# fixie-ai/ultravox

Hardware: NVIDIA H100
Metric: audio-sec/s prefill (Llama-3.1-8B, 30s clip) at 1/2/4/8 H100; TTFT p50 (higher is better)
Workload: dtype bf16

## Files before the change

### ultravox_b200/csrc/gemm_tc.cu

```cuda
#include <stdlib.h>

#include "uvx_common.cuh"
#include "tc_ptx.cuh"

namespace uvx {

struct GemmParams {
  int64_t a_rows, a_batch, K, N;
  void* C;
  int64_t c_row_stride, c_batch_rows, c_row_offset;
  const int32_t* c_row_map;
  const bf16* bias;
  const bf16* R;
  int64_t r_row_stride, r_batch_stride;
  float alpha;
  int act, out_f32;
  int m_tiles;
  int n_tiles, num_tiles;
  int splits, kb_per_split;
  float* ws_partial;
  const bf16* norm_w;
  bf16* norm_out;
  float norm_eps;
  int w_tiled;
  int w_perm;
  int swiglu;
  const float* rope_cos;
  const float* rope_sin;
  const int32_t* rope_pos;
  int64_t rope_rows_per_seq, rope_pos_offset;
  int rope_cols;
  int stages;
  int cm, cn;
};

static constexpr int kSmemTotal = 227 * 1024;
static constexpr int kMaxStages = 8;
static constexpr int kGemmThreads = 384;

template <int MT, int BN>
struct WgLayout {
  static constexpr int kABytes = MT * 128 * kBK * 2;
  static constexpr int kWBytes = BN * kBK * 2;
  static constexpr int kStageBytes = kABytes + kWBytes;
  static constexpr int kRingMax = kSmemTotal - 1024 - 256;
  static constexpr int kStages = kRingMax / kStageBytes > kMaxStages ? kMaxStages : kRingMax / kStageBytes;
  static constexpr int kAcc = BN / 2;
  static_assert(kStages >= 2, "ring too shallow");
  static_assert(MT * kAcc <= 128, "accumulators must fit the register file");
};

__device__ __forceinline__ int tile_col(int tc, int perm) {
  if (!perm) return tc;
  const int q = tc >> 5, j = tc & 31;
  return j < 16 ? 16 * q + j : 64 + 16 * q + (j - 16);
}

__device__ __forceinline__ int64_t out_row(const GemmParams& p, int b, int64_t m) {
  return p.c_row_map ? (int64_t)p.c_row_map[(int64_t)b * p.a_rows + m] : (int64_t)b * p.c_batch_rows + m + p.c_row_offset;
}

template <int BN, int I>
__device__ __forceinline__ void swiglu_row(const GemmParams& p, const float* a, int h, int cq, bf16* crow, int64_t n_out0) {
#pragma unroll
  for (int j = 0; j < BN / 8; ++j) {
    if ((8 * j) % (2 * I) >= I) continue;
    const int64_t f = n_out0 + (8 * j / (2 * I)) * I + (8 * j) % (2 * I) + cq;
    if (f >= p.N / 2) continue;
    constexpr int kUp = I / 8;
    float o[2];
#pragma unroll
    for (int e = 0; e < 2; ++e) {
      const float gate = __bfloat162float(__float2bfloat16_rn(a[4 * j + 2 * h + e] * p.alpha));
      const float up = __bfloat162float(__float2bfloat16_rn(a[4 * (j + kUp) + 2 * h + e] * p.alpha));
      o[e] = __bfloat162float(__float2bfloat16_rn(silu_fast(gate))) * up;
    }
    *reinterpret_cast<__nv_bfloat162*>(crow + f) = __floats2bfloat162_rn(o[0], o[1]);
  }
}

__device__ __forceinline__ void rope_store(const GemmParams& p, float x1a, float x1b, float x2a, float x2b, int64_t pos, int d, bf16* crow) {
  const float2 cs = *reinterpret_cast<const float2*>(p.rope_cos + pos * 64 + d);
  const float2 sn = *reinterpret_cast<const float2*>(p.rope_sin + pos * 64 + d);
  float o1a, o2a, o1b, o2b;
  rope_pair(__bfloat162float(__float2bfloat16_rn(x1a * p.alpha)), __bfloat162float(__float2bfloat16_rn(x2a * p.alpha)), cs.x, sn.x, o1a, o2a);
  rope_pair(__bfloat162float(__float2bfloat16_rn(x1b * p.alpha)), __bfloat162float(__float2bfloat16_rn(x2b * p.alpha)), cs.y, sn.y, o1b, o2b);
  *reinterpret_cast<__nv_bfloat162*>(crow + d) = __floats2bfloat162_rn(o1a, o1b);
  *reinterpret_cast<__nv_bfloat162*>(crow + d + 64) = __floats2bfloat162_rn(o2a, o2b);
}

template <int MT, int BN>
__global__ void __launch_bounds__(kGemmThreads, 1)
gemm_wg_kernel(const __grid_constant__ CUtensorMap tmA, const __grid_constant__ CUtensorMap tmW, const GemmParams p) {
  using L = WgLayout<MT, BN>;
  pdl_trigger();
  extern __shared__ uint8_t smem_raw[];
  uint8_t* smem = (uint8_t*)(((uintptr_t)smem_raw + 1023) & ~(uintptr_t)1023);
  uint64_t* full_bar = (uint64_t*)(smem + p.stages * L::kStageBytes);
  uint64_t* empty_bar = full_bar + kMaxStages;

  const int wg = threadIdx.x >> 7, tid = threadIdx.x & 127;
  const int tiles_m_total = p.m_tiles * (int)p.a_batch;
  const int num_kb = (int)((p.K + kBK - 1) / kBK);
  const int stages = p.stages;
  const int csize = p.cm * p.cn;
  const int rank = csize > 1 ? (int)cluster_ctarank() : 0;
  const int rm = rank / p.cn, rn = rank % p.cn;
  const int cluster_tiles_m = tiles_m_total / p.cm;
  const int num_units = p.num_tiles / csize * p.splits;
  const int first_unit = blockIdx.x / csize, unit_step = gridDim.x / csize;

  if (threadIdx.x == 0) {
    for (int s = 0; s < stages; ++s) {
      mbar_init(&full_bar[s], 1);
      mbar_init(&empty_bar[s], 8 * csize);
    }
    asm volatile("fence.mbarrier_init.release.cluster;" ::: "memory");
    asm volatile("fence.proxy.async.shared::cta;" ::: "memory");
  }
  if (csize > 1) cluster_sync();
  else __syncthreads();
  pdl_wait();

  if (wg == 0) {
    asm volatile("setmaxnreg.dec.sync.aligned.u32 40;");
    if (tid == 0) {
      asm volatile("prefetch.tensormap [%0];" ::"l"(&tmA) : "memory");
      asm volatile("prefetch.tensormap [%0];" ::"l"(&tmW) : "memory");
      const int a_slice = MT * 128 / p.cn, w_slice = BN / p.cm;
      const uint16_t row_mask = (uint16_t)(((1u << p.cn) - 1u) << (rm * p.cn));
      uint16_t col_mask = 0;
      for (int j = 0; j < p.cm; ++j) col_mask |= (uint16_t)(1u << (j * p.cn + rn));
      int s = 0;
      uint32_t ph = 0;
      for (int unit = first_unit; unit < num_units; unit += unit_step) {
        const int ctile = unit / p.splits, split = unit % p.splits;
        const int tm_idx = (ctile % cluster_tiles_m) * p.cm + rm;
        const int tn_idx = (ctile / cluster_tiles_m) * p.cn + rn;
        const int b = tm_idx / p.m_tiles;
        const int m0 = (tm_idx % p.m_tiles) * (MT * 128);
        const int kb_begin = split * p.kb_per_split;
        const int kb_end = min(num_kb, kb_begin + p.kb_per_split);
        const int wt_base = tn_idx * num_kb * BN;
        for (int kb = kb_begin; kb < kb_end; ++kb) {
          mbar_wait(&empty_bar[s], ph ^ 1u);
          uint8_t* sa = smem + s * L::kStageBytes;
          mbar_expect_tx(&full_bar[s], (uint32_t)L::kStageBytes);
          uint8_t* da = sa + rn * a_slice * (kBK * 2);
          if (p.cn > 1) tma_load_3d_mc(da, &tmA, kb * kBK, m0 + rn * a_slice, b, &full_bar[s], row_mask);
          else tma_load_3d(da, &tmA, kb * kBK, m0, b, &full_bar[s]);
          uint8_t* dw = sa + L::kABytes + rm * w_slice * (kBK * 2);
          const int w0 = p.w_tiled ? 0 : kb * kBK;
          const int w1 = (p.w_tiled ? wt_base + kb * BN : tn_idx * BN) + rm * w_slice;
          if (p.cm > 1) tma_load_2d_mc(dw, &tmW, w0, w1, &full_bar[s], col_mask);
          else tma_load_2d(dw, &tmW, w0, w1, &full_bar[s]);
          if (++s == stages) { s = 0; ph ^= 1u; }
        }
      }
    }
    if (csize > 1) cluster_sync();
    return;
  }

  asm volatile("setmaxnreg.inc.sync.aligned.u32 232;");
  const int c = wg - 1;
  const int warp = tid >> 5, lane = tid & 31;
  auto release = [&](int slot) {
    __syncwarp();
    if (csize == 1) {
      if (lane == 0) mbar_arrive(&empty_bar[slot]);
    } else if (lane < csize) {
// ... 25 lines not shown
#pragma unroll
        for (int k = 0; k < kBK / 16; ++k)
          Wgmma<BN>::mma(acc[mt], da + (uint64_t)(2 * k), dw + (uint64_t)(2 * k), (kb > kb_begin || k > 0) ? 1u : 0u);
      }
      wgmma_commit();
      wgmma_wait<1>();
      if (prev >= 0) release(prev);
      prev = s;
      if (++s == stages) { s = 0; ph ^= 1u; }
    }
    wgmma_wait<0>();
    release(prev);

    const int rq = warp * 16 + (lane >> 2);
    const int cq = 2 * (lane & 3);
    if (p.splits > 1) {
      float* part = p.ws_partial + (size_t)split * (size_t)(p.a_batch * p.a_rows) * (size_t)p.N;
#pragma unroll
      for (int mt = 0; mt < MT; ++mt) {
#pragma unroll
        for (int h = 0; h < 2; ++h) {
          const int64_t m = (int64_t)m0 + mt * 128 + c * 64 + rq + 8 * h;
          if (m >= p.a_rows) continue;
          float* dst = part + ((size_t)b * p.a_rows + m) * p.N;
#pragma unroll
          for (int j = 0; j < BN / 8; ++j) {
            const int64_t n = n0 + tile_col(8 * j + cq, p.w_perm);
            if (n < p.N) *reinterpret_cast<float2*>(dst + n) = make_float2(acc[mt][4 * j + 2 * h], acc[mt][4 * j + 2 * h + 1]);
          }
        }
      }
      continue;
    }
    if (p.swiglu) {
      const int64_t n_out0 = (int64_t)tn_idx * (BN / 2);
#pragma unroll
      for (int mt = 0; mt < MT; ++mt) {
#pragma unroll
        for (int h = 0; h < 2; ++h) {
          const int64_t m = (int64_t)m0 + mt * 128 + c * 64 + rq + 8 * h;
          if (m >= p.a_rows) continue;
          const int64_t orow = out_row(p, b, m);
          if (orow < 0) continue;
          bf16* crow = reinterpret_cast<bf16*>(p.C) + orow * p.c_row_stride;
          if (p.swiglu == 16) swiglu_row<BN, 16>(p, acc[mt], h, cq, crow, n_out0);
          else swiglu_row<BN, 8>(p, acc[mt], h, cq, crow, n_out0);
        }
      }
      continue;
    }
    if constexpr (BN == 128) {
      if (p.rope_cos != nullptr && n0 < p.rope_cols) {
#pragma unroll
        for (int mt = 0; mt < MT; ++mt) {
#pragma unroll
          for (int h = 0; h < 2; ++h) {
            const int64_t m = (int64_t)m0 + mt * 128 + c * 64 + rq + 8 * h;
            if (m >= p.a_rows) continue;
            const int64_t orow = out_row(p, b, m);
            if (orow < 0) continue;
            const int64_t pos = p.rope_pos ? (int64_t)p.rope_pos[m] : p.rope_pos_offset + (m % p.rope_rows_per_seq);
            bf16* crow = reinterpret_cast<bf16*>(p.C) + orow * p.c_row_stride + n0;
            const float* a = acc[mt];
            if (!p.w_perm) {
#pragma unroll
              for (int j = 0; j < 8; ++j)
                rope_store(p, a[4 * j + 2 * h], a[4 * j + 2 * h + 1], a[4 * (j + 8) + 2 * h], a[4 * (j + 8) + 2 * h + 1], pos, 8 * j + cq, crow);
            } else {
#pragma unroll
              for (int q = 0; q < 4; ++q)
#pragma unroll
                for (int jj = 0; jj < 2; ++jj) {
                  const int j = 4 * q + jj;
                  rope_store(p, a[4 * j + 2 * h], a[4 * j + 2 * h + 1], a[4 * (j + 2) + 2 * h], a[4 * (j + 2) + 2 * h + 1], pos,
                             16 * q + 8 * jj + cq, crow);
                }
            }
          }
        }
        continue;
      }
    }
#pragma unroll
    for (int mt = 0; mt < MT; ++mt) {
#pragma unroll
      for (int h = 0; h < 2; ++h) {
        const int64_t m = (int64_t)m0 + mt * 128 + c * 64 + rq + 8 * h;
        if (m >= p.a_rows) continue;
        const int64_t orow = out_row(p, b, m);
        if (orow < 0) continue;
        const bf16* rrow = p.R ? p.R + (int64_t)b * p.r_batch_stride + m * p.r_row_stride : nullptr;
#pragma unroll
        for (int j = 0; j < BN / 8; ++j) {
          const int64_t n = n0 + tile_col(8 * j + cq, p.w_perm);
          if (n >= p.N) continue;
          float v0 = acc[mt][4 * j + 2 * h] * p.alpha, v1 = acc[mt][4 * j + 2 * h + 1] * p.alpha;
          if (p.bias) {
            const float2 t = __bfloat1622float2(*reinterpret_cast<const __nv_bfloat162*>(p.bias + n));
            v0 += t.x;
            v1 += t.y;
          }
          if (p.act == UVX_ACT_GELU) {
            v0 = gelu_fast(v0);
            v1 = gelu_fast(v1);
          }
          if (rrow) {
            const float2 t = __bfloat1622float2(*reinterpret_cast<const __nv_bfloat162*>(rrow + n));
            v0 += t.x;
            v1 += t.y;
          }
          if (p.out_f32)
            *reinterpret_cast<float2*>(reinterpret_cast<float*>(p.C) + orow * p.c_row_stride + n) = make_float2(v0, v1);
          else
            *reinterpret_cast<__nv_bfloat162*>(reinterpret_cast<bf16*>(p.C) + orow * p.c_row_stride + n) = __floats2bfloat162_rn(v0, v1);
        }
      }
    }
  }
  if (csize > 1) cluster_sync();
}

__global__ void __launch_bounds__(256) splitk_reduce_kernel(const GemmParams p) {
  pdl_trigger();
  pdl_wait();
  const int64_t rows = p.a_batch * p.a_rows;
  const int64_t vec_per_row = p.N / 8;
  const int64_t total = rows * vec_per_row;
  const size_t split_stride = (size_t)rows * (size_t)p.N;
  for (int64_t idx = (int64_t)blockIdx.x * blockDim.x + threadIdx.x; idx < total; idx += (int64_t)gridDim.x * blockDim.x) {
    const int64_t r = idx / vec_per_row, n = (idx % vec_per_row) * 8;
    const int64_t b = r / p.a_rows, m = r % p.a_rows;
    const float* src = p.ws_partial + (size_t)r * p.N + n;
    float v[8] = {0.f, 0.f, 0.f, 0.f, 0.f, 0.f, 0.f, 0.f};
#pragma unroll 4
    for (int sidx = 0; sidx < p.splits; ++sidx) {
      const float4 t0 = __ldcg(reinterpret_cast<const float4*>(src + sidx * split_stride));
      const float4 t1 = __ldcg(reinterpret_cast<const float4*>(src + sidx * split_stride) + 1);
      v[0] += t0.x; v[1] += t0.y; v[2] += t0.z; v[3] += t0.w;
      v[4] += t1.x; v[5] += t1.y; v[6] += t1.z; v[7] += t1.w;
    }
    const int64_t orow = p.c_row_map ? (int64_t)p.c_row_map[r] : b * p.c_batch_rows + m + p.c_row_offset;
    if (orow < 0) continue;
#pragma unroll
    for (int i = 0; i < 8; ++i) v[i] *= p.alpha;
    if (p.bias) {
      float t[8];
      unpack8(*reinterpret_cast<const bf16x8*>(p.bias + n), t);
#pragma unroll
      for (int i = 0; i < 8; ++i) v[i] += t[i];
    }
    if (p.act == UVX_ACT_GELU) {
#pragma unroll
      for (int i = 0; i < 8; ++i) v[i] = gelu_erf(v[i]);
    }
    if (p.R) {
      float t[8];
      unpack8(*reinterpret_cast<const bf16x8*>(p.R + b * p.r_batch_stride + m * p.r_row_stride + n), t);
#pragma unroll
      for (int i = 0; i < 8; ++i) v[i] += t[i];
    }
    if (p.out_f32) {
      float4* dst = reinterpret_cast<float4*>(reinterpret_cast<float*>(p.C) + orow * p.c_row_stride + n);
      dst[0] = make_float4(v[0], v[1], v[2], v[3]);
      dst[1] = make_float4(v[4], v[5], v[6], v[7]);
    } else {
      *reinterpret_cast<bf16x8*>(reinterpret_cast<bf16*>(p.C) + orow * p.c_row_stride + n) = pack8(v);
    }
  }
}

__global__ void __launch_bounds__(256) splitk_reduce_rmsnorm_kernel(const GemmParams p) {
  pdl_trigger();
  pdl_wait();
  __shared__ float red[32];
  const int64_t r = blockIdx.x;
  const int64_t b = r / p.a_rows, m = r % p.a_rows;
  const int64_t rows = p.a_batch * p.a_rows;
  const size_t split_stride = (size_t)rows * (size_t)p.N;
  const int64_t orow = p.c_row_map ? (int64_t)p.c_row_map[r] : b * p.c_batch_rows + m + p.c_row_offset;
  constexpr int kMaxV = 4;
  float v[kMaxV][8];
  float sq = 0.f;
  const int nvec = (int)(p.N / 8);
#pragma unroll
  for (int i = 0; i < kMaxV; ++i) {
    const int j = threadIdx.x + i * 256;
    if (j < nvec) {
      const int64_t n = (int64_t)j * 8;
      const float* src = p.ws_partial + (size_t)r * p.N + n;
#pragma unroll
      for (int e = 0; e < 8; ++e) v[i][e] = 0.f;
      for (int s0 = 0; s0 < p.splits; s0 += 4) {
        float4 t0[4], t1[4];
#pragma unroll
        for (int u = 0; u < 4; ++u) {
          if (s0 + u < p.splits) {
            t0[u] = __ldcg(reinterpret_cast<const float4*>(src + (s0 + u) * split_stride));
            t1[u] = __ldcg(reinterpret_cast<const float4*>(src + (s0 + u) * split_stride) + 1);
          }
        }
#pragma unroll
        for (int u = 0; u < 4; ++u) {
// ... 179 lines not shown
}

typedef CUresult (*EncodeTiledFn)(CUtensorMap*, CUtensorMapDataType, cuuint32_t, void*, const cuuint64_t*,
                                  const cuuint64_t*, const cuuint32_t*, const cuuint32_t*, CUtensorMapInterleave,
                                  CUtensorMapSwizzle, CUtensorMapL2promotion, CUtensorMapFloatOOBfill);

static EncodeTiledFn get_encode() {
  static EncodeTiledFn fn = nullptr;
  if (!fn) {
    void* p = nullptr;
    cudaDriverEntryPointQueryResult q;
    if (cudaGetDriverEntryPoint("cuTensorMapEncodeTiled", &p, cudaEnableDefault, &q) == cudaSuccess &&
        q == cudaDriverEntryPointSuccess)
      fn = (EncodeTiledFn)p;
  }
  return fn;
}

static int encode_map(CUtensorMap* tm, const void* base, int rank, const uint64_t* dims, const uint64_t* strides_bytes,
                      const uint32_t* box, CUtensorMapL2promotion promo) {
  EncodeTiledFn enc = get_encode();
  if (!enc) {
    set_error("cuTensorMapEncodeTiled entry point not available");
    return UVX_ERR_CUDA;
  }
  cuuint64_t gd[3];
  cuuint64_t gs[2];
  cuuint32_t bx[3], es[3];
  for (int i = 0; i < rank; ++i) {
    gd[i] = dims[i];
    bx[i] = box[i];
    es[i] = 1;
  }
  for (int i = 0; i < rank - 1; ++i) gs[i] = strides_bytes[i];
  CUresult r = enc(tm, CU_TENSOR_MAP_DATA_TYPE_BFLOAT16, (cuuint32_t)rank, const_cast<void*>(base), gd, gs, bx, es,
                   CU_TENSOR_MAP_INTERLEAVE_NONE, CU_TENSOR_MAP_SWIZZLE_128B, promo, CU_TENSOR_MAP_FLOAT_OOB_FILL_NONE);
  if (r != CUDA_SUCCESS) {
    set_error("cuTensorMapEncodeTiled failed with CUresult %d (rank %d dims %llu %llu stride %llu)", (int)r, rank,
              (unsigned long long)dims[0], (unsigned long long)dims[1], (unsigned long long)strides_bytes[0]);
    return UVX_ERR_CUDA;
  }
  return UVX_OK;
}

static int num_sms() {
  static int n = 0;
  if (!n) {
    int dev = 0;
    cudaGetDevice(&dev);
    cudaDeviceGetAttribute(&n, cudaDevAttrMultiProcessorCount, dev);
    if (n <= 0) n = 132;
  }
  return n;
}

static int g_gemm_stage_cap = 0;
static int g_grid_cap = 0;

static int finish_gemm(const uvx_gemm_args* a, const GemmParams& p, cudaStream_t stream) {
  const bool want_norm = a->norm_w && a->norm_out;
  if (p.splits == 1) {
    if (!want_norm) return UVX_OK;
    return uvx_rmsnorm(a->C, a->norm_w, a->norm_out, a->a_batch * a->a_rows, a->N, a->c_row_stride, 0, 0, 0, a->norm_eps, stream);
  }
  if (want_norm && !p.out_f32 && a->N <= 8192 && !a->c_row_map && a->act == UVX_ACT_NONE) {
    launch_k(splitk_reduce_rmsnorm_kernel, dim3((unsigned)(a->a_batch * a->a_rows)), dim3(256), 0, stream, p);
    return check_launch("splitk_reduce_rmsnorm_kernel");
  }
  const int64_t total = a->a_batch * a->a_rows * (a->N / 8);
  int64_t blocks = (total + 255) / 256;
  if (blocks > (int64_t)num_sms() * 8) blocks = (int64_t)num_sms() * 8;
  launch_k(splitk_reduce_kernel, dim3((unsigned)blocks), dim3(256), 0, stream, p);
  int rc = check_launch("splitk_reduce_kernel");
  if (rc || !want_norm) return rc;
  return uvx_rmsnorm(a->C, a->norm_w, a->norm_out, a->a_batch * a->a_rows, a->N, a->c_row_stride, 0, 0, 0, a->norm_eps, stream);
}

static void legal_cluster(int mt, int bn, int tiles_m_total, int n_tiles, int* cm, int* cn) {
  if (*cm < 1 || *cm > 4 || tiles_m_total % *cm != 0 || bn % (8 * *cm) != 0) *cm = 1;
  if (*cn < 1 || *cn > 4 || n_tiles % *cn != 0 || (mt * 128) % (8 * *cn) != 0) *cn = 1;
  if (*cm * *cn > 8) *cm = *cn = 1;
}

template <int MT, int BN>
static int launch_gemm(const uvx_gemm_args* a, int splits, int cm, int cn, cudaStream_t stream) {
  using L = WgLayout<MT, BN>;
  const int m_tiles = (int)((a->a_rows + MT * 128 - 1) / (MT * 128));
  const int n_tiles = (int)((a->N + BN - 1) / BN);
  legal_cluster(MT, BN, m_tiles * (int)a->a_batch, n_tiles, &cm, &cn);
  CUtensorMap tmA, tmW;
  {
    uint64_t dims[3] = {(uint64_t)a->K, (uint64_t)a->a_rows, (uint64_t)a->a_batch};
    uint64_t st[2] = {(uint64_t)a->a_row_stride * 2, (uint64_t)(a->a_batch > 1 ? a->a_batch_stride : a->a_row_stride) * 2};
    uint32_t box[3] = {kBK, (uint32_t)(MT * 128 / cn), 1};
    int rc = encode_map(&tmA, a->A, 3, dims, st, box, CU_TENSOR_MAP_L2_PROMOTION_L2_128B);
    if (rc) return rc;
  }
  const bool tiled = a->w_tiled != 0;
  if (tiled) {
    UVX_REQUIRE(a->w_tiled == BN && a->K % kBK == 0, "uvx_gemm_bf16: tiled weights need BN == tile rows and K %% 64 == 0");
    const uint64_t n_tiles_w = (uint64_t)((a->N + BN - 1) / BN);
    uint64_t dims[2] = {(uint64_t)kBK, n_tiles_w * (uint64_t)(a->K / kBK) * (uint64_t)BN};
    uint64_t st[1] = {(uint64_t)kBK * 2};
    uint32_t box[2] = {kBK, (uint32_t)(BN / cm)};
    int rc = encode_map(&tmW, a->W, 2, dims, st, box, CU_TENSOR_MAP_L2_PROMOTION_L2_256B);
    if (rc) return rc;
  } else {
    uint64_t dims[2] = {(uint64_t)a->K, (uint64_t)a->N};
    uint64_t st[1] = {(uint64_t)a->w_row_stride * 2};
    uint32_t box[2] = {kBK, (uint32_t)(BN / cm)};
    int rc = encode_map(&tmW, a->W, 2, dims, st, box, CU_TENSOR_MAP_L2_PROMOTION_L2_256B);
    if (rc) return rc;
  }
  GemmParams p;
  memset(&p, 0, sizeof(p));
  p.w_tiled = tiled ? 1 : 0;
  p.w_perm = a->w_perm == 1 ? 1 : 0;
  p.swiglu = a->act == UVX_ACT_SWIGLU ? (a->w_tiled == 128 ? 16 : 8) : 0;
  p.rope_cos = a->rope_cos;
  p.rope_sin = a->rope_sin;
  p.rope_pos = a->rope_positions;
  p.rope_rows_per_seq = a->rope_rows_per_seq > 0 ? a->rope_rows_per_seq : 1;
  p.rope_pos_offset = a->rope_pos_offset;
  p.rope_cols = a->rope_cos ? (int)a->rope_cols : 0;
  if (p.swiglu || p.rope_cos || p.w_perm) splits = 1;
  p.a_rows = a->a_rows;
  p.a_batch = a->a_batch;
  p.K = a->K;
  p.N = a->N;
  p.C = a->C;
  p.c_row_stride = a->c_row_stride;
  p.c_batch_rows = a->c_batch_rows;
  p.c_row_offset = a->c_row_offset;
  p.c_row_map = a->c_row_map;
  p.bias = (const bf16*)a->bias;
  p.R = (const bf16*)a->R;
  p.r_row_stride = a->r_row_stride;
  p.r_batch_stride = a->r_batch_stride;
  p.alpha = a->alpha;
  p.act = a->act;
  p.out_f32 = a->out_dtype == UVX_DT_F32;
  p.norm_w = (const bf16*)a->norm_w;
  p.norm_out = (bf16*)a->norm_out;
  p.norm_eps = a->norm_eps;
  p.m_tiles = m_tiles;
  p.n_tiles = n_tiles;
  p.num_tiles = p.m_tiles * (int)a->a_batch * p.n_tiles;
  p.cm = cm;
  p.cn = cn;
  const int num_kb = (int)((a->K + kBK - 1) / kBK);
  if (a->N % BN != 0) splits = 1;
  const size_t per_split = (size_t)a->a_batch * (size_t)a->a_rows * (size_t)a->N * 4;
  while (splits > 1 && (!a->workspace || per_split * (size_t)splits > (size_t)a->workspace_bytes)) --splits;
  if (splits > num_kb) splits = num_kb;
  if (splits < 1) splits = 1;
  p.kb_per_split = (num_kb + splits - 1) / splits;
  p.splits = (num_kb + p.kb_per_split - 1) / p.kb_per_split;
  p.ws_partial = (float*)a->workspace;
  p.stages = L::kStages;
  if (g_gemm_stage_cap >= 2 && p.stages > g_gemm_stage_cap) p.stages = g_gemm_stage_cap;
  const int smem = p.stages * L::kStageBytes + 1024 + 2 * kMaxStages * 8;
  static bool attr_set = false;
  if (!attr_set) {
    cudaError_t e = cudaFuncSetAttribute(gemm_wg_kernel<MT, BN>, cudaFuncAttributeMaxDynamicSharedMemorySize, kSmemTotal);
    if (e != cudaSuccess) {
      set_error("cudaFuncSetAttribute(gemm_wg_kernel<%d,%d>, smem %d): %s", MT, BN, kSmemTotal, cudaGetErrorString(e));
      return UVX_ERR_CUDA;
    }
    attr_set = true;
  }
  const int csize = cm * cn;
  const int units = p.num_tiles / csize * p.splits;
  int max_units = num_sms();
  if (csize > 1) {
    static int max_clusters[9] = {0};
    if (!max_clusters[csize]) {
      cudaLaunchConfig_t cfg = {};
      cfg.gridDim = dim3((unsigned)csize);
      cfg.blockDim = dim3(kGemmThreads);
      cfg.dynamicSmemBytes = (size_t)smem;
      cudaLaunchAttribute attr;
      attr.id = cudaLaunchAttributeClusterDimension;
      attr.val.clusterDim.x = (unsigned)csize;
      attr.val.clusterDim.y = 1;
      attr.val.clusterDim.z = 1;
      cfg.attrs = &attr;
      cfg.numAttrs = 1;
      cudaError_t e = cudaOccupancyMaxActiveClusters(&max_clusters[csize], gemm_wg_kernel<MT, BN>, &cfg);
      if (e != cudaSuccess || max_clusters[csize] < 1) {
        set_error("cudaOccupancyMaxActiveClusters(gemm_wg_kernel<%d,%d>, %d CTAs): %s", MT, BN, csize,
                  e != cudaSuccess ? cudaGetErrorString(e) : "no cluster fits");
        max_clusters[csize] = 0;
        return UVX_ERR_CUDA;
      }
    }
    max_units = max_clusters[csize];
  }
  int clusters = units < max_units ? units : max_units;
  if (g_grid_cap > 0 && clusters * csize > g_grid_cap) clusters = g_grid_cap / csize > 1 ? g_grid_cap / csize : 1;
  const dim3 grid((unsigned)(clusters * csize));
  if (csize > 1)
    launch_k_cluster(gemm_wg_kernel<MT, BN>, grid, dim3(kGemmThreads), (size_t)smem, stream, (unsigned)csize, tmA, tmW, p);
  else
    launch_k(gemm_wg_kernel<MT, BN>, grid, dim3(kGemmThreads), (size_t)smem, stream, tmA, tmW, p);
  int rc = check_launch("gemm_wg_kernel");
  if (rc) return rc;
  return finish_gemm(a, p, stream);
}

static int g_ws_enable = -1;

static int gemm_ws_enabled() {
  if (g_ws_enable < 0) {
    const char* e = getenv("UVX_GEMM_WS");
    g_ws_enable = e ? atoi(e) : 2;
  }
  return g_ws_enable;
}

static bool gemm_ws_common(const uvx_gemm_args* a) {
  if (!gemm_ws_enabled() || (a->flags & 2)) return false;
  if (a->a_batch != 1 || a->out_dtype != UVX_DT_BF16 || a->c_row_map || a->c_row_offset != 0) return false;
  return a->w_tiled == 0 || a->w_tiled == 128;
}

static bool gemm_swap_eligible(const uvx_gemm_args* a) {
  if (!gemm_ws_common(a) || a->a_rows > 32 || a->act == UVX_ACT_SWIGLU) return false;
  return a->workspace && (size_t)a->workspace_bytes >= (size_t)a->a_rows * (size_t)a->N * 4;
}

static bool gemm_ws_eligible(const uvx_gemm_args* a) {
  return gemm_ws_common(a) && gemm_ws_enabled() == 1 && a->a_rows <= 256 && a->N % 128 == 0;
}

template <int BT>
static int launch_gemm_swap(const uvx_gemm_args* a, cudaStream_t stream) {
  constexpr int kStage = 128 * kBK * 2 + BT * kBK * 2;
  CUtensorMap tmX, tmW;
  {
    uint64_t dims[2] = {(uint64_t)a->K, (uint64_t)a->a_rows};
    uint64_t st[1] = {(uint64_t)a->a_row_stride * 2};
    uint32_t box[2] = {kBK, (uint32_t)BT};
    int rc = encode_map(&tmX, a->A, 2, dims, st, box, CU_TENSOR_MAP_L2_PROMOTION_L2_128B);
    if (rc) return rc;
  }
  const int num_kb = (int)((a->K + kBK - 1) / kBK);
  const int n_tiles = (int)((a->N + 127) / 128);
  if (a->w_tiled) {
    UVX_REQUIRE(a->K % kBK == 0, "uvx_gemm_bf16: tiled weights need K %% 64 == 0");
    uint64_t dims[2] = {(uint64_t)kBK, (uint64_t)n_tiles * (uint64_t)num_kb * 128};
    uint64_t st[1] = {(uint64_t)kBK * 2};
    uint32_t box[2] = {kBK, 128};
    int rc = encode_map(&tmW, a->W, 2, dims, st, box, CU_TENSOR_MAP_L2_PROMOTION_L2_256B);
    if (rc) return rc;
  } else {
    uint64_t dims[2] = {(uint64_t)a->K, (uint64_t)a->N};
    uint64_t st[1] = {(uint64_t)a->w_row_stride * 2};
    uint32_t box[2] = {kBK, 128};
    int rc = encode_map(&tmW, a->W, 2, dims, st, box, CU_TENSOR_MAP_L2_PROMOTION_L2_256B);
    if (rc) return rc;
  }
  GemmParams p;
  memset(&p, 0, sizeof(p));
  p.a_rows = a->a_rows;
  p.a_batch = 1;
  p.K = a->K;
  p.N = a->N;
  p.C = a->C;
  p.c_row_stride = a->c_row_stride;
  p.c_batch_rows = a->a_rows;
  p.bias = (const bf16*)a->bias;
  p.R = (const bf16*)a->R;
  p.r_row_stride = a->r_row_stride;
  p.r_batch_stride = a->r_batch_stride;
  p.alpha = a->alpha;
  p.act = a->act;
  p.norm_w = (const bf16*)a->norm_w;
  p.norm_out = (bf16*)a->norm_out;
  p.norm_eps = a->norm_eps;
  p.w_tiled = a->w_tiled ? 1 : 0;
  p.w_perm = a->w_perm == 1 ? 1 : 0;
  p.rope_cos = a->rope_cos;
  p.rope_sin = a->rope_sin;
  p.rope_pos = a->rope_positions;
  p.rope_rows_per_seq = a->rope_rows_per_seq > 0 ? a->rope_rows_per_seq : 1;
  p.rope_pos_offset = a->rope_pos_offset;
  p.rope_cols = a->rope_cos ? (int)a->rope_cols : 0;
  p.n_tiles = n_tiles;
  p.num_tiles = n_tiles;
  const int sms = num_sms();
  int splits = 1;
  if (n_tiles * 2 <= sms && num_kb >= 16) {
    splits = sms / n_tiles;
    if (splits > num_kb / 8) splits = num_kb / 8;
    if (splits > 16) splits = 16;
    if (splits < 1) splits = 1;
  }
  if (a->N % 8 != 0) splits = 1;
  const size_t per_split = (size_t)a->a_rows * (size_t)a->N * 4;
  while (splits > 1 && per_split * (size_t)splits > (size_t)a->workspace_bytes) --splits;
  p.kb_per_split = (num_kb + splits - 1) / splits;
  p.splits = (num_kb + p.kb_per_split - 1) / p.kb_per_split;
  p.ws_partial = (float*)a->workspace;
  p.stages = (kSmemTotal - 1024 - 256) / kStage;
  if (p.stages > kMaxStages) p.stages = kMaxStages;
  if (g_gemm_stage_cap >= 2 && p.stages > g_gemm_stage_cap) p.stages = g_gemm_stage_cap;
  const int smem = p.stages * kStage + 1024 + 2 * kMaxStages * 8;
  static bool attr_set = false;
  if (!attr_set) {
    cudaError_t e = cudaFuncSetAttribute(gemm_swap_kernel<BT>, cudaFuncAttributeMaxDynamicSharedMemorySize, kSmemTotal);
    if (e != cudaSuccess) {
      set_error("cudaFuncSetAttribute(gemm_swap_kernel<%d>): %s", BT, cudaGetErrorString(e));
      return UVX_ERR_CUDA;
    }
    attr_set = true;
  }
  const int units = n_tiles * p.splits;
  int grid = units < sms ? units : sms;
  if (g_grid_cap > 0 && grid > g_grid_cap) grid = g_grid_cap;
  launch_k(gemm_swap_kernel<BT>, dim3((unsigned)grid), dim3(kGemmThreads), (size_t)smem, stream, tmX, tmW, p);
  int rc = check_launch("gemm_swap_kernel");
  if (rc) return rc;
  if (p.rope_cos) {
    const int64_t total = a->a_rows * (a->N / 128) * 8;
    const int64_t blocks = (total + 255) / 256;
    launch_k(splitk_reduce_rope_kernel, dim3((unsigned)blocks), dim3(256), 0, stream, p);
    return check_launch("splitk_reduce_rope_kernel");
  }
  return finish_gemm(a, p, stream);
}

}

static int forced = -1, forced_splits = -1;

extern "C" int uvx_debug_gemm_override(int cfg, int splits) {
  forced = cfg;
  forced_splits = splits;
  return UVX_OK;
}

extern "C" int uvx_debug_gemm_stages(int n) {
  uvx::g_gemm_stage_cap = n;
  return UVX_OK;
}

extern "C" int uvx_debug_gemm_ws(int enable, int mode, int grid) {
  (void)mode;
  uvx::g_ws_enable = enable;
  uvx::g_grid_cap = grid > 0 ? grid : 0;
  return UVX_OK;
}

static int forced_cm = 0, forced_cn = 0;
static int g_cluster_enable = -1;

extern "C" int uvx_debug_gemm_cluster(int cm, int cn) {
  forced_cm = cm;
  forced_cn = cn;
  return UVX_OK;
}

extern "C" int uvx_debug_gemm_mode(int mode) { (void)mode; return UVX_OK; }
extern "C" int uvx_debug_gemm_tma_store(int on) { (void)on; return UVX_OK; }
extern "C" int uvx_debug_gemm_times(void* dev_buf) { (void)dev_buf; return UVX_OK; }
extern "C" int uvx_debug_gemm_pf(int pf) { (void)pf; return UVX_OK; }
extern "C" int uvx_debug_gemm_ws_times(void* dev_buf) { (void)dev_buf; return UVX_OK; }

static void read_forced() {
  if (forced < 0) {
    const char* e = getenv("UVX_GEMM_CFG");
    forced = e ? atoi(e) : 0;
    const char* s = getenv("UVX_GEMM_SPLITS");
    forced_splits = s ? atoi(s) : 0;
  }
}

static void pick_cfg(int64_t rows, int64_t batch, int64_t N, int64_t K, int sms, int* mt_out, int* bn_out, int* splits) {
  const int num_kb = (int)((K + 63) / 64);
  int mt, bn;
  if (rows <= 256 && batch == 1) {
    mt = rows > 128 ? 2 : 1;
    bn = N % 128 == 0 ? 128 : 64;
    if (bn == 128 && 2 * (N / 128) >= (sms * 3) / 5 && N / 128 < sms && num_kb <= 80) mt = 1;
  } else {
    mt = 1;
    const int64_t m_tiles = (rows + 127) / 128 * batch;
    if (N % 256 == 0 && m_tiles * (N / 256) >= sms && num_kb >= 32) bn = 256;
    else bn = (N % 128 == 0 && m_tiles * (N / 128) >= sms / 2) ? 128 : 64;
  }
  const int64_t tiles = ((rows + mt * 128 - 1) / (mt * 128)) * batch * ((N + bn - 1) / bn);
  int sp = 1;
  if (tiles * 2 <= sms && num_kb >= 16) {
    sp = (int)(sms / tiles);
    if (sp > num_kb / 8) sp = num_kb / 8;
    if (sp > 16) sp = 16;
    if (sp < 1) sp = 1;
  }
  *mt_out = mt;
  *bn_out = bn;
  *splits = sp;
}

static void pick_cluster(int64_t rows, int64_t batch, int mt, int* cm, int* cn) {
  *cm = *cn = 1;
  if (g_cluster_enable < 0) {
    const char* e = getenv("UVX_GEMM_CLUSTER");
    g_cluster_enable = e ? atoi(e) : 1;
  }
  if (forced_cm > 0 || forced_cn > 0) {
    *cm = forced_cm > 0 ? forced_cm : 1;
    *cn = forced_cn > 0 ? forced_cn : 1;
    return;
  }
  if (!g_cluster_enable || rows > 256 || batch != 1) return;
  if (mt == 1 && rows > 128) {
    *cm = 2;
    *cn = 2;
  }
}

extern "C" int uvx_gemm_bf16(const uvx_gemm_args* a, uvx_stream_t stream_) {
  using namespace uvx;
  cudaStream_t stream = (cudaStream_t)stream_;
  UVX_REQUIRE(a && a->A && a->W && a->C, "uvx_gemm_bf16: null pointer");
  UVX_REQUIRE(a->a_batch >= 1 && a->a_rows >= 1 && a->K >= 8 && a->N >= 64, "uvx_gemm_bf16: empty problem");
  UVX_REQUIRE(a->K % 8 == 0 && a->N % 64 == 0, "uvx_gemm_bf16: K %% 8 and N %% 64 required (K=%lld N=%lld)",
              (long long)a->K, (long long)a->N);
  UVX_REQUIRE(a->a_row_stride % 8 == 0 && a->w_row_stride % 8 == 0 && (a->a_batch == 1 || a->a_batch_stride % 8 == 0),
              "uvx_gemm_bf16: strides must be multiples of 8 elements");
  UVX_REQUIRE(((uintptr_t)a->A % 16 == 0) && ((uintptr_t)a->W % 16 == 0) && ((uintptr_t)a->C % 16 == 0),
              "uvx_gemm_bf16: 16-byte aligned bases required");
  UVX_REQUIRE(a->c_row_stride % 8 == 0 && (!a->R || (a->r_row_stride % 8 == 0 && a->r_batch_stride % 8 == 0)),
              "uvx_gemm_bf16: output / residual strides must be multiples of 8");
  UVX_REQUIRE(a->a_rows < (1ll << 31) && a->K < (1ll << 31) && a->N < (1ll << 31), "uvx_gemm_bf16: dimension too large");
  UVX_REQUIRE(!a->workspace || (uintptr_t)a->workspace % 256 == 0, "uvx_gemm_bf16: workspace must be 256-byte aligned");
  UVX_REQUIRE(!(a->norm_w && a->norm_out) || (a->out_dtype == UVX_DT_BF16 && !a->c_row_map && a->c_row_offset == 0 &&
                                              (a->a_batch == 1 || a->c_batch_rows == a->a_rows)),
              "uvx_gemm_bf16: fused RMSNorm needs a plain bf16 output");
  UVX_REQUIRE(a->w_tiled == 0 || a->w_tiled == 64 || a->w_tiled == 128 || a->w_tiled == 208 || a->w_tiled == 256,
              "uvx_gemm_bf16: w_tiled must be 64 / 128 / 208 / 256");
  UVX_REQUIRE(a->w_perm == 0 || (a->w_perm == 1 && a->w_tiled == 128 && a->N % 128 == 0 && a->act != UVX_ACT_SWIGLU),
              "uvx_gemm_bf16: the pair-permuted image (w_perm = 1) is a 128-row image of whole heads");
  UVX_REQUIRE(a->act != UVX_ACT_SWIGLU || (a->w_tiled != 0 && !a->bias && !a->R && !a->norm_w && a->out_dtype == UVX_DT_BF16 &&
                                           a->N % (a->w_tiled == 128 ? 32 : 16) == 0),
              "uvx_gemm_bf16: UVX_ACT_SWIGLU needs the interleaved gate|up image, bf16 output, no bias / residual / norm");
  UVX_REQUIRE(!a->rope_cos || (a->rope_sin && a->a_batch == 1 && a->alpha == 1.0f && !a->bias && !a->R && a->act == UVX_ACT_NONE &&
                               a->rope_cols % 128 == 0 && (a->w_tiled == 0 || a->w_tiled == 128) && a->N % 128 == 0),
              "uvx_gemm_bf16: fused RoPE needs head_dim 128 tiles, a_batch 1, no bias / residual / activation");
  read_forced();
  const int sms = num_sms();
  int mt, bn, splits;
  pick_cfg(a->a_rows, a->a_batch, a->N, a->K, sms, &mt, &bn, &splits);
  if (forced <= 0 && forced_splits <= 0 && gemm_swap_eligible(a)) {
    if (a->a_rows <= 8) return launch_gemm_swap<8>(a, stream);
    if (a->a_rows <= 16) return launch_gemm_swap<16>(a, stream);
    return launch_gemm_swap<32>(a, stream);
  }
  const bool ws = forced <= 0 && forced_splits <= 0 && gemm_ws_eligible(a);
  if (ws) {
    mt = 1;
    bn = 128;
    splits = 1;
  } else if (forced > 0) {
    const int fb = forced % 1000, fm = forced / 1000;
    if (fb == 64 || fb == 128 || fb == 208 || fb == 256) {
      if (a->N % fb == 0 || fb == 208) bn = fb;
      mt = fm == 2 ? 2 : 1;
    }
  }
  if (forced_splits > 0 && !ws) splits = forced_splits;
  if (a->w_tiled) bn = (int)a->w_tiled;
  if (a->rope_cos) {
    mt = 1;
    bn = 128;
  }
  if (bn > 128) mt = 1;
  int cm, cn;
  pick_cluster(a->a_rows, a->a_batch, mt, &cm, &cn);
  switch (mt * 1000 + bn) {
    case 1064: return launch_gemm<1, 64>(a, splits, cm, cn, stream);
    case 1128: return launch_gemm<1, 128>(a, splits, cm, cn, stream);
    case 1208: return launch_gemm<1, 208>(a, splits, cm, cn, stream);
    case 1256: return launch_gemm<1, 256>(a, splits, cm, cn, stream);
    case 2064: return launch_gemm<2, 64>(a, splits, cm, cn, stream);
    case 2128: return launch_gemm<2, 128>(a, splits, cm, cn, stream);
    default: return launch_gemm<1, 64>(a, splits, cm, cn, stream);
  }
}
```

Before: 1411.

## Add ping-pong warp-specialized GEMM kernel with heuristic tile selection

Adds a persistent GEMM kernel in which two consumer warpgroups alternate between output tiles, ordered by named barriers, so one warpgroup's epilogue overlaps the other's MMA main loop. A single TMA producer warpgroup feeds a shared smem ring. A heuristic picks 64x256 or 128x128 tiles when the per-SM wave work is lower than the cooperative kernel's, and only for plain GEMMs (no SwiGLU, RoPE, tiled weights or split-K). The plain epilogue is factored into a shared helper. Risks include extra register pressure from per-warpgroup accumulators and wrong pipeline phase tracking if the tile interleaving assumptions break.

```diff
diff --git a/ultravox_b200/csrc/gemm_tc.cu b/ultravox_b200/csrc/gemm_tc.cu
--- a/ultravox_b200/csrc/gemm_tc.cu
+++ b/ultravox_b200/csrc/gemm_tc.cu
@@ -87,6 +87,42 @@
   rope_pair(__bfloat162float(__float2bfloat16_rn(x1b * p.alpha)), __bfloat162float(__float2bfloat16_rn(x2b * p.alpha)), cs.y, sn.y, o1b, o2b);
   *reinterpret_cast<__nv_bfloat162*>(crow + d) = __floats2bfloat162_rn(o1a, o1b);
   *reinterpret_cast<__nv_bfloat162*>(crow + d + 64) = __floats2bfloat162_rn(o2a, o2b);
+}
+
+template <int BN>
+__device__ __forceinline__ void plain_epilogue(const GemmParams& p, const float* acc, int b, int64_t m_sub0, int n0, int rq, int cq) {
+#pragma unroll
+  for (int h = 0; h < 2; ++h) {
+    const int64_t m = m_sub0 + rq + 8 * h;
+    if (m >= p.a_rows) continue;
+    const int64_t orow = out_row(p, b, m);
+    if (orow < 0) continue;
+    const bf16* rrow = p.R ? p.R + (int64_t)b * p.r_batch_stride + m * p.r_row_stride : nullptr;
+#pragma unroll
+    for (int j = 0; j < BN / 8; ++j) {
+      const int64_t n = n0 + tile_col(8 * j + cq, p.w_perm);
+      if (n >= p.N) continue;
+      float v0 = acc[4 * j + 2 * h] * p.alpha, v1 = acc[4 * j + 2 * h + 1] * p.alpha;
+      if (p.bias) {
+        const float2 t = __bfloat1622float2(*reinterpret_cast<const __nv_bfloat162*>(p.bias + n));
+        v0 += t.x;
+        v1 += t.y;
+      }
+      if (p.act == UVX_ACT_GELU) {
+        v0 = gelu_fast(v0);
+        v1 = gelu_fast(v1);
+      }
+      if (rrow) {
+        const float2 t = __bfloat1622float2(*reinterpret_cast<const __nv_bfloat162*>(rrow + n));
+        v0 += t.x;
+        v1 += t.y;
+      }
+      if (p.out_f32)
+        *reinterpret_cast<float2*>(reinterpret_cast<float*>(p.C) + orow * p.c_row_stride + n) = make_float2(v0, v1);
+      else
+        *reinterpret_cast<__nv_bfloat162*>(reinterpret_cast<bf16*>(p.C) + orow * p.c_row_stride + n) = __floats2bfloat162_rn(v0, v1);
+    }
+  }
 }
 
 template <int MT, int BN>
@@ -278,42 +314,127 @@
       }
     }
 #pragma unroll
-    for (int mt = 0; mt < MT; ++mt) {
-#pragma unroll
-      for (int h = 0; h < 2; ++h) {
-        const int64_t m = (int64_t)m0 + mt * 128 + c * 64 + rq + 8 * h;
-        if (m >= p.a_rows) continue;
-        const int64_t orow = out_row(p, b, m);
-        if (orow < 0) continue;
-        const bf16* rrow = p.R ? p.R + (int64_t)b * p.r_batch_stride + m * p.r_row_stride : nullptr;
-#pragma unroll
-        for (int j = 0; j < BN / 8; ++j) {
-          const int64_t n = n0 + tile_col(8 * j + cq, p.w_perm);
-          if (n >= p.N) continue;
-          float v0 = acc[mt][4 * j + 2 * h] * p.alpha, v1 = acc[mt][4 * j + 2 * h + 1] * p.alpha;
-          if (p.bias) {
-            const float2 t = __bfloat1622float2(*reinterpret_cast<const __nv_bfloat162*>(p.bias + n));
-            v0 += t.x;
-            v1 += t.y;
-          }
-          if (p.act == UVX_ACT_GELU) {
-            v0 = gelu_fast(v0);
-            v1 = gelu_fast(v1);
-          }
-          if (rrow) {
-            const float2 t = __bfloat1622float2(*reinterpret_cast<const __nv_bfloat162*>(rrow + n));
-            v0 += t.x;
-            v1 += t.y;
-          }
-          if (p.out_f32)
-            *reinterpret_cast<float2*>(reinterpret_cast<float*>(p.C) + orow * p.c_row_stride + n) = make_float2(v0, v1);
-          else
-            *reinterpret_cast<__nv_bfloat162*>(reinterpret_cast<bf16*>(p.C) + orow * p.c_row_stride + n) = __floats2bfloat162_rn(v0, v1);
+    for (int mt = 0; mt < MT; ++mt) plain_epilogue<BN>(p, acc[mt], b, (int64_t)m0 + mt * 128 + c * 64, n0, rq, cq);
+  }
+  if (csize > 1) cluster_sync();
+}
+
+template <int TM, int TN>
+struct PpLayout {
+  static constexpr int kABytes = TM * kBK * 2;
+  static constexpr int kWBytes = TN * kBK * 2;
+  static constexpr int kStageBytes = kABytes + kWBytes;
+  static constexpr int kRingMax = kSmemTotal - 1024 - 256;
+  static constexpr int kStages = kRingMax / kStageBytes > kMaxStages ? kMaxStages : kRingMax / kStageBytes;
+  static constexpr int kSub = TM / 64;
+  static constexpr int kAcc = TN / 2;
+  static_assert(kStages >= 2, "ring too shallow");
+  static_assert(kSub * kAcc <= 128, "accumulators must fit the register file");
+};
+
+__device__ __forceinline__ void named_bar_sync(int id, int threads) {
+  asm volatile("bar.sync %0, %1;" ::"r"(id), "r"(threads) : "memory");
+}
+__device__ __forceinline__ void named_bar_arrive(int id, int threads) {
+  asm volatile("bar.arrive %0, %1;" ::"r"(id), "r"(threads) : "memory");
+}
+
+template <int TM, int TN>
+__global__ void __launch_bounds__(kGemmThreads, 1)
+gemm_pp_kernel(const __grid_constant__ CUtensorMap tmA, const __grid_constant__ CUtensorMap tmW, const GemmParams p) {
+  using L = PpLayout<TM, TN>;
+  pdl_trigger();
+  extern __shared__ uint8_t smem_raw[];
+  uint8_t* smem = (uint8_t*)(((uintptr_t)smem_raw + 1023) & ~(uintptr_t)1023);
+  uint64_t* full_bar = (uint64_t*)(smem + p.stages * L::kStageBytes);
+  uint64_t* empty_bar = full_bar + kMaxStages;
+
+  const int wg = threadIdx.x >> 7, tid = threadIdx.x & 127;
+  const int tiles_m_total = p.m_tiles * (int)p.a_batch;
+  const int num_kb = (int)((p.K + kBK - 1) / kBK);
+  const int stages = p.stages;
+  const int n_local = (p.num_tiles - (int)blockIdx.x + (int)gridDim.x - 1) / (int)gridDim.x;
+
+  if (threadIdx.x == 0) {
+    for (int s = 0; s < stages; ++s) {
+      mbar_init(&full_bar[s], 1);
+      mbar_init(&empty_bar[s], 4);
+    }
+    asm volatile("fence.mbarrier_init.release.cluster;" ::: "memory");
+    asm volatile("fence.proxy.async.shared::cta;" ::: "memory");
+  }
+  __syncthreads();
+  pdl_wait();
+
+  if (wg == 0) {
+    asm volatile("setmaxnreg.dec.sync.aligned.u32 40;");
+    if (tid == 0) {
+      asm volatile("prefetch.tensormap [%0];" ::"l"(&tmA) : "memory");
+      asm volatile("prefetch.tensormap [%0];" ::"l"(&tmW) : "memory");
+      int s = 0;
+      uint32_t ph = 0;
+      for (int i = 0; i < n_local; ++i) {
+        const int t = (int)blockIdx.x + i * (int)gridDim.x;
+        const int tm_idx = t % tiles_m_total, tn_idx = t / tiles_m_total;
+        const int b = tm_idx / p.m_tiles;
+        const int m0 = (tm_idx % p.m_tiles) * TM;
+        for (int kb = 0; kb < num_kb; ++kb) {
+          mbar_wait(&empty_bar[s], ph ^ 1u);
+          uint8_t* sa = smem + s * L::kStageBytes;
+          mbar_expect_tx(&full_bar[s], (uint32_t)L::kStageBytes);
+          tma_load_3d(sa, &tmA, kb * kBK, m0, b, &full_bar[s]);
+          tma_load_2d(sa + L::kABytes, &tmW, kb * kBK, tn_idx * TN, &full_bar[s]);
+          if (++s == stages) { s = 0; ph ^= 1u; }
         }
       }
     }
-  }
-  if (csize > 1) cluster_sync();
+    return;
+  }
+
+  asm volatile("setmaxnreg.inc.sync.aligned.u32 232;");
+  const int c = wg - 1;
+  const int warp = tid >> 5, lane = tid & 31;
+  const int rq = warp * 16 + (lane >> 2), cq = 2 * (lane & 3);
+  for (int i = c; i < n_local; i += 2) {
+    const int t = (int)blockIdx.x + i * (int)gridDim.x;
+    const int tm_idx = t % tiles_m_total, tn_idx = t / tiles_m_total;
+    const int b = tm_idx / p.m_tiles;
+    const int m0 = (tm_idx % p.m_tiles) * TM;
+    const int n0 = tn_idx * TN;
+    const int pos = i * num_kb;
+    int s = pos % stages;
+    uint32_t ph = (uint32_t)((pos / stages) & 1);
+    if (i > 0) named_bar_sync(1 + c, 256);
+    float acc[L::kSub][L::kAcc];
+    int prev = -1;
+    for (int kb = 0; kb < num_kb; ++kb) {
+      mbar_wait(&full_bar[s], ph);
+      const uint32_t sa = smem_u32(smem + s * L::kStageBytes);
+      const uint64_t dw = make_wgmma_desc(sa + L::kABytes);
+      wgmma_fence();
+#pragma unroll
+      for (int sub = 0; sub < L::kSub; ++sub) {
+        const uint64_t da = make_wgmma_desc(sa + sub * 64 * (kBK * 2));
+#pragma unroll
+        for (int k = 0; k < kBK / 16; ++k)
+          Wgmma<TN>::mma(acc[sub], da + (uint64_t)(2 * k), dw + (uint64_t)(2 * k), (kb > 0 || k > 0) ? 1u : 0u);
+      }
+      wgmma_commit();
+      wgmma_wait<1>();
+      if (prev >= 0) {
+        __syncwarp();
+        if (lane == 0) mbar_arrive(&empty_bar[prev]);
+      }
+      prev = s;
+      if (++s == stages) { s = 0; ph ^= 1u; }
+    }
+    if (i + 1 < n_local) named_bar_arrive(2 - c, 256);
+    wgmma_wait<0>();
+    __syncwarp();
+    if (lane == 0) mbar_arrive(&empty_bar[prev]);
+#pragma unroll
+    for (int sub = 0; sub < L::kSub; ++sub) plain_epilogue<TN>(p, acc[sub], b, (int64_t)m0 + sub * 64, n0, rq, cq);
+  }
 }
 
 __global__ void __launch_bounds__(256) splitk_reduce_kernel(const GemmParams p) {
@@ -659,6 +780,43 @@
   if (*cm * *cn > 8) *cm = *cn = 1;
 }
 
+static int encode_a_map(CUtensorMap* tm, const uvx_gemm_args* a, int box_rows) {
+  uint64_t dims[3] = {(uint64_t)a->K, (uint64_t)a->a_rows, (uint64_t)a->a_batch};
+  uint64_t st[2] = {(uint64_t)a->a_row_stride * 2, (uint64_t)(a->a_batch > 1 ? a->a_batch_stride : a->a_row_stride) * 2};
+  uint32_t box[3] = {kBK, (uint32_t)box_rows, 1};
+  return encode_map(tm, a->A, 3, dims, st, box, CU_TENSOR_MAP_L2_PROMOTION_L2_128B);
+}
+
+static int encode_w_map(CUtensorMap* tm, const uvx_gemm_args* a, int box_rows) {
+  uint64_t dims[2] = {(uint64_t)a->K, (uint64_t)a->N};
+  uint64_t st[1] = {(uint64_t)a->w_row_stride * 2};
+  uint32_t box[2] = {kBK, (uint32_t)box_rows};
+  return encode_map(tm, a->W, 2, dims, st, box, CU_TENSOR_MAP_L2_PROMOTION_L2_256B);
+}
+
+static void plain_params(const uvx_gemm_args* a, GemmParams* p) {
+  memset(p, 0, sizeof(*p));
+  p->a_rows = a->a_rows;
+  p->a_batch = a->a_batch;
+  p->K = a->K;
+  p->N = a->N;
+  p->C = a->C;
+  p->c_row_stride = a->c_row_stride;
+  p->c_batch_rows = a->c_batch_rows;
+  p->c_row_offset = a->c_row_offset;
+  p->c_row_map = a->c_row_map;
+  p->bias = (const bf16*)a->bias;
+  p->R = (const bf16*)a->R;
+  p->r_row_stride = a->r_row_stride;
+  p->r_batch_stride = a->r_batch_stride;
+  p->alpha = a->alpha;
+  p->act = a->act;
+  p->out_f32 = a->out_dtype == UVX_DT_F32;
+  p->norm_w = (const bf16*)a->norm_w;
+  p->norm_out = (bf16*)a->norm_out;
+  p->norm_eps = a->norm_eps;
+}
+
 template <int MT, int BN>
 static int launch_gemm(const uvx_gemm_args* a, int splits, int cm, int cn, cudaStream_t stream) {
   using L = WgLayout<MT, BN>;
@@ -667,10 +825,7 @@
   legal_cluster(MT, BN, m_tiles * (int)a->a_batch, n_tiles, &cm, &cn);
   CUtensorMap tmA, tmW;
   {
-    uint64_t dims[3] = {(uint64_t)a->K, (uint64_t)a->a_rows, (uint64_t)a->a_batch};
-    uint64_t st[2] = {(uint64_t)a->a_row_stride * 2, (uint64_t)(a->a_batch > 1 ? a->a_batch_stride : a->a_row_stride) * 2};
-    uint32_t box[3] = {kBK, (uint32_t)(MT * 128 / cn), 1};
-    int rc = encode_map(&tmA, a->A, 3, dims, st, box, CU_TENSOR_MAP_L2_PROMOTION_L2_128B);
+    int rc = encode_a_map(&tmA, a, MT * 128 / cn);
     if (rc) return rc;
   }
   const bool tiled = a->w_tiled != 0;
@@ -683,14 +838,11 @@
     int rc = encode_map(&tmW, a->W, 2, dims, st, box, CU_TENSOR_MAP_L2_PROMOTION_L2_256B);
     if (rc) return rc;
   } else {
-    uint64_t dims[2] = {(uint64_t)a->K, (uint64_t)a->N};
-    uint64_t st[1] = {(uint64_t)a->w_row_stride * 2};
-    uint32_t box[2] = {kBK, (uint32_t)(BN / cm)};
-    int rc = encode_map(&tmW, a->W, 2, dims, st, box, CU_TENSOR_MAP_L2_PROMOTION_L2_256B);
+    int rc = encode_w_map(&tmW, a, BN / cm);
     if (rc) return rc;
   }
   GemmParams p;
-  memset(&p, 0, sizeof(p));
+  plain_params(a, &p);
   p.w_tiled = tiled ? 1 : 0;
   p.w_perm = a->w_perm == 1 ? 1 : 0;
   p.swiglu = a->act == UVX_ACT_SWIGLU ? (a->w_tiled == 128 ? 16 : 8) : 0;
@@ -701,25 +853,6 @@
   p.rope_pos_offset = a->rope_pos_offset;
   p.rope_cols = a->rope_cos ? (int)a->rope_cols : 0;
   if (p.swiglu || p.rope_cos || p.w_perm) splits = 1;
-  p.a_rows = a->a_rows;
-  p.a_batch = a->a_batch;
-  p.K = a->K;
-  p.N = a->N;
-  p.C = a->C;
-  p.c_row_stride = a->c_row_stride;
-  p.c_batch_rows = a->c_batch_rows;
-  p.c_row_offset = a->c_row_offset;
-  p.c_row_map = a->c_row_map;
-  p.bias = (const bf16*)a->bias;
-  p.R = (const bf16*)a->R;
-  p.r_row_stride = a->r_row_stride;
-  p.r_batch_stride = a->r_batch_stride;
-  p.alpha = a->alpha;
-  p.act = a->act;
-  p.out_f32 = a->out_dtype == UVX_DT_F32;
-  p.norm_w = (const bf16*)a->norm_w;
-  p.norm_out = (bf16*)a->norm_out;
-  p.norm_eps = a->norm_eps;
   p.m_tiles = m_tiles;
   p.n_tiles = n_tiles;
   p.num_tiles = p.m_tiles * (int)a->a_batch * p.n_tiles;
@@ -781,6 +914,42 @@
   else
     launch_k(gemm_wg_kernel<MT, BN>, grid, dim3(kGemmThreads), (size_t)smem, stream, tmA, tmW, p);
   int rc = check_launch("gemm_wg_kernel");
+  if (rc) return rc;
+  return finish_gemm(a, p, stream);
+}
+
+template <int TM, int TN>
+static int launch_gemm_pp(const uvx_gemm_args* a, cudaStream_t stream) {
+  using L = PpLayout<TM, TN>;
+  CUtensorMap tmA, tmW;
+  int rc = encode_a_map(&tmA, a, TM);
+  if (rc) return rc;
+  rc = encode_w_map(&tmW, a, TN);
+  if (rc) return rc;
+  GemmParams p;
+  plain_params(a, &p);
+  p.m_tiles = (int)((a->a_rows + TM - 1) / TM);
+  p.n_tiles = (int)((a->N + TN - 1) / TN);
+  p.num_tiles = p.m_tiles * (int)a->a_batch * p.n_tiles;
+  p.cm = p.cn = 1;
+  p.splits = 1;
+  p.kb_per_split = (int)((a->K + kBK - 1) / kBK);
+  p.stages = L::kStages;
+  if (g_gemm_stage_cap >= 2 && p.stages > g_gemm_stage_cap) p.stages = g_gemm_stage_cap;
+  const int smem = p.stages * L::kStageBytes + 1024 + 2 * kMaxStages * 8;
+  static bool attr_set = false;
+  if (!attr_set) {
+    cudaError_t e = cudaFuncSetAttribute(gemm_pp_kernel<TM, TN>, cudaFuncAttributeMaxDynamicSharedMemorySize, kSmemTotal);
+    if (e != cudaSuccess) {
+      set_error("cudaFuncSetAttribute(gemm_pp_kernel<%d,%d>, smem %d): %s", TM, TN, kSmemTotal, cudaGetErrorString(e));
+      return UVX_ERR_CUDA;
+    }
+    attr_set = true;
+  }
+  int grid = p.num_tiles < num_sms() ? p.num_tiles : num_sms();
+  if (g_grid_cap > 0 && grid > g_grid_cap) grid = g_grid_cap;
+  launch_k(gemm_pp_kernel<TM, TN>, dim3((unsigned)grid), dim3(kGemmThreads), (size_t)smem, stream, tmA, tmW, p);
+  rc = check_launch("gemm_pp_kernel");
   if (rc) return rc;
   return finish_gemm(a, p, stream);
 }
@@ -938,7 +1107,13 @@
   return UVX_OK;
 }
 
-extern "C" int uvx_debug_gemm_mode(int mode) { (void)mode; return UVX_OK; }
+static int g_pp_mode = -1;
+
+extern "C" int uvx_debug_gemm_mode(int mode) {
+  g_pp_mode = mode;
+  return UVX_OK;
+}
+
 extern "C" int uvx_debug_gemm_tma_store(int on) { (void)on; return UVX_OK; }
 extern "C" int uvx_debug_gemm_times(void* dev_buf) { (void)dev_buf; return UVX_OK; }
 extern "C" int uvx_debug_gemm_pf(int pf) { (void)pf; return UVX_OK; }
@@ -995,6 +1170,32 @@
     *cm = 2;
     *cn = 2;
   }
+}
+
+static int pick_pp(const uvx_gemm_args* a, int sms, int mt, int bn, int splits) {
+  if (g_pp_mode < 0) {
+    const char* e = getenv("UVX_GEMM_PP");
+    g_pp_mode = e ? atoi(e) : 0;
+  }
+  const int mode = g_pp_mode;
+  if (mode == 1) return 0;
+  if (a->a_rows <= 256 && a->a_batch == 1) return 0;
+  if (a->act == UVX_ACT_SWIGLU || a->rope_cos || a->w_tiled || a->w_perm) return 0;
+  if ((forced_splits > 0 ? forced_splits : splits) > 1 || forced_cm > 1 || forced_cn > 1) return 0;
+  if (mode == 3) return 64256;
+  if (mode == 4) return 128128;
+  const bool wide = a->N % 256 == 0 && a->K >= 1024;
+  const int tile = wide ? 64256 : 128128;
+  if (mode == 2) return tile;
+  if (forced > 0 || forced_splits > 0) return 0;
+  const int64_t tm = wide ? 64 : 128, tn = wide ? 256 : 128;
+  const int64_t pp_tiles = (a->a_rows + tm - 1) / tm * a->a_batch * ((a->N + tn - 1) / tn);
+  const int64_t coop_tiles = (a->a_rows + mt * 128 - 1) / (mt * 128) * a->a_batch * ((a->N + bn - 1) / bn);
+  if (pp_tiles <= sms) return 0;
+  const int64_t pp_work = (pp_tiles + sms - 1) / sms * tm * tn;
+  const int64_t coop_work = (coop_tiles + sms - 1) / sms * mt * 128 * bn;
+  if (pp_work < coop_work) return tile;
+  return pp_work == coop_work && mt * bn <= 128 && a->K >= 4096 ? tile : 0;
 }
 
 extern "C" int uvx_gemm_bf16(const uvx_gemm_args* a, uvx_stream_t stream_) {
@@ -1034,6 +1235,11 @@
     if (a->a_rows <= 16) return launch_gemm_swap<16>(a, stream);
     return launch_gemm_swap<32>(a, stream);
   }
+  switch (pick_pp(a, sms, mt, bn, splits)) {
+    case 64256: return launch_gemm_pp<64, 256>(a, stream);
+    case 128128: return launch_gemm_pp<128, 128>(a, stream);
+    default: break;
+  }
   const bool ws = forced <= 0 && forced_splits <= 0 && gemm_ws_eligible(a);
   if (ws) {
     mt = 1;
```

After: 1413, median of 6. Within noise of the previous version (+0.2%).
